# mrjoshuak/go-jpeg2000

Hardware: AMD Instinct MI355X
Metric: Mpixels/s encode+decode (4K sRGB, 5-3 lossless) (higher is better)
Workload: dtype int32

## Files before the change

### go-jpeg2000_amd/csrc/ht.hip

```cpp
#include <cstdlib>

#include "ht_tables.h"
#include "j2k_internal.h"

namespace j2k {

__device__ __constant__ uint16_t c_vlc_tbl0[1024] = J2K_HT_VLC_TBL0_INIT;
__device__ __constant__ uint16_t c_vlc_tbl1[1024] = J2K_HT_VLC_TBL1_INIT;
__device__ uint16_t g_vlc_enc[2 * 4 * 16];

__global__ void ht_build_enc_table() {
    const int t = threadIdx.x;
    if (t >= 128) return;
    const int initial = t >> 6, context = (t >> 4) & 3, rho = t & 15;
    const uint16_t *tbl = initial ? c_vlc_tbl0 : c_vlc_tbl1;
    uint16_t r = 0x0001;
    for (uint32_t cwd = 0; cwd < 128; cwd++) {
        const uint16_t e = tbl[(context << 7) | cwd];
        if (((e >> 4) & 0xF) == rho && (e & 0xF) > 0) { r = (uint16_t)((cwd << 4) | (e & 0xF)); break; }
    }
    g_vlc_enc[t] = r;
}

__device__ uint16_t g_vlc_pair1[16384];
// ... 813 lines not shown
    for (long i = 0; i < num && size > 0; i++) {
        if (unstuff && pos < len && data[pos] > 0x8F) return false;
        uint32_t b;
        if (size > 0 && pos < len) { b = data[pos]; pos++; size--; } else b = 0xFF;
        if (size == 1) b |= 0x0F;
        unstuff = (b == 0xFF);
    }
    return true;
}

#define HT_WALK_MAX_PAIRS 128
#define HT_DEC_MWORDS (33 * HT_FAST_MAX_SAMPLES / 32 + 8)
#define HT_WALK_REC 132
#define HT_PAIR_SERIAL 0xFFFFFFFFu
#define HT_PAIR_ZERO 0xFFFFFFFEu

__device__ __forceinline__ void wave_sync() {
    __builtin_amdgcn_fence(__ATOMIC_RELEASE, "wavefront");
    __builtin_amdgcn_wave_barrier();
    __builtin_amdgcn_fence(__ATOMIC_ACQUIRE, "wavefront");
}

__device__ __forceinline__ uint32_t get_bits32(const uint32_t *buf, uint32_t bitpos) {
    const uint32_t wd = bitpos >> 5, sh = bitpos & 31;
    const uint64_t two = (uint64_t)buf[wd] | ((uint64_t)buf[wd + 1] << 32);
    return (uint32_t)(two >> sh);
}

__device__ __forceinline__ uint32_t get_bits32_cut(const uint32_t *buf, uint32_t bitpos, uint32_t L) {
    if (bitpos >= L) return 0;
    const uint32_t p = bitpos < (HT_DEC_MWORDS - 2) * 32u ? bitpos : (HT_DEC_MWORDS - 2) * 32u + (bitpos & 31);
    uint32_t v = get_bits32(buf, p);
    if (L - bitpos < 32) v &= (1u << (L - bitpos)) - 1;
    return v;
}

#define HT_VBITS_WORDS 192
#define HT_VROW 193

__global__ __launch_bounds__(256) void ht_vlcprep_kernel(const BlockJob *__restrict__ jobs, int njobs,
                                                         const uint8_t *__restrict__ stream, const uint64_t *__restrict__ offs,
                                                         const uint32_t *__restrict__ lens, uint32_t *__restrict__ vbits,
                                                         uint32_t *__restrict__ pairs) {
    __shared__ uint32_t vb4[4][HT_VBITS_WORDS + 8];
    uint32_t *vb = vb4[threadIdx.x >> 6];
    const int jid = blockIdx.x * 4 + (threadIdx.x >> 6);
    if (jid >= njobs) return;
    const int lane = threadIdx.x & 63;
    const int w = jobs[jid].w, h = jobs[jid].h;
    const long len = (long)lens[jid];
    const uint8_t *data = stream + offs[jid];
    uint32_t *rec = pairs + (size_t)jid * HT_WALK_REC;
    const int quadCols = (w + 3) / 4, P = (quadCols + 1) / 2, R = (h + 3) / 4, N = R * P;
    const bool fast = (size_t)R * (size_t)w <= HT_FAST_MAX_SAMPLES && N <= HT_WALK_MAX_PAIRS;
    uint32_t tag = 0;
    long scup = 0;
    if (!fast) tag = HT_PAIR_SERIAL;
    else if (len < 2) tag = HT_PAIR_ZERO;
    else {
        scup = (long)data[len - 1] + ((long)(data[len - 2] & 0x0F) << 8);
        if (scup < 2 || scup > len) tag = HT_PAIR_ZERO;
        else if (!init_mel_ok(data, len, len, scup)) tag = HT_PAIR_ZERO;
    }
    if (tag) {
        if (lane == 0) { rec[0] = tag; rec[HT_WALK_MAX_PAIRS] = 0; }
        return;
    }
    for (int i = lane; i < HT_VBITS_WORDS + 8; i += 64) vb[i] = 0;
    wave_sync();
    const long lcup = len;
    const uint32_t b0 = data[lcup - 2];
    const uint32_t t0 = b0 >> 4;
    uint32_t off = 4 - ((t0 & 7) >> 2);
    if (lane == 0) atomicOr(&vb[0], t0);
    const long size = scup - 2;
    const long maxbytes = (long)(46 * N + 7) / 8 + 8;
    const long nb = size < maxbytes ? size : maxbytes;
    uint32_t carry = b0 | 0x0F;
    for (long k0 = 1; k0 <= nb; k0 += 256) {
        const long k = k0 + 4 * lane;
        const long e = lcup - 2 - k;
        uint32_t dw = 0;
// ... 76 lines not shown
#pragma unroll
        for (int j = 0; j < 8; j++) reinterpret_cast<uint4 *>(S.pair1)[j * 256 + tid] = t[j];
#pragma unroll
        for (int j = 0; j < NV; j++) {
            const int q = j * 256 + tid;
            uint32_t *d = &S.vb[q / 48][4 * (q % 48)];
            d[0] = v[j].x; d[1] = v[j].y; d[2] = v[j].z; d[3] = v[j].w;
        }
    }
    __syncthreads();
#ifdef J2K_WALK_STAMP
    const long long st1 = __builtin_amdgcn_s_memtime();
#endif
    if (tid >= 64) return;
    const int quadCols = (w + 3) / 4, P = (quadCols + 1) / 2, R = (h + 3) / 4;
    const bool walks = have && tag != HT_PAIR_SERIAL && tag != HT_PAIR_ZERO;
    int nsteps = walks ? R * P : 0;
#pragma unroll
    for (int o = 32; o > 0; o >>= 1) nsteps = max(nsteps, __shfl_xor(nsteps, o));
    nsteps = min(__builtin_amdgcn_readfirstlane(nsteps), HT_WALK_MAX_PAIRS);
    if (!walks) return;
    const uint32_t *row = &S.vb[lane][0];
    uint32_t pos = 0;
#define HT_FETCH(w0, w1)                                                          \
    uint32_t w0, w1;                                                               \
    {                                                                              \
        const uint32_t *p_ = row + (pos >> 5);                                     \
        const uint32_t d0_ = p_[0], d1_ = p_[1], d2_ = p_[2];                      \
        w0 = __builtin_amdgcn_alignbit(d1_, d0_, pos & 31);                        \
        w1 = __builtin_amdgcn_alignbit(d2_, d1_, pos & 31);                        \
    }
// ... 64 lines not shown
};

__device__ uint32_t ht_loaded_bits(const HtDecShared &S, uint32_t nff, long segLen, uint32_t j) {
    const long k = 4 * (long)j;
    const long kk = k < segLen ? k : segLen;
    uint32_t f = 0, last_ff = 0;
    for (uint32_t i = 0; i < nff; i++) {
        if ((long)S.ffpos[i] + 2 <= kk) f++;
        if ((long)S.ffpos[i] == segLen - 1) last_ff = 1;
    }
    uint32_t b = (uint32_t)(8 * kk) - f;
    if (k > segLen) b += (last_ff ? 7u : 8u) + 7u * (uint32_t)(k - segLen - 1);
    return b;
}

template <bool STRIDED>
__device__ bool ht_extract_fast(HtDecShared &S, const uint8_t *__restrict__ data, long len, long scup, int w, int h,
                                int32_t *__restrict__ out, int lane, bool bigu, const uint32_t (&mpos2)[2], uint32_t total_bits,
                                const uint32_t (&raw0)[4], int os_) {
    const size_t os64 = STRIDED ? (size_t)os_ : (size_t)64, osw = STRIDED ? (size_t)os_ : (size_t)w;
    const int quadCols = (w + 3) / 4, P = (quadCols + 1) / 2, R = (h + 3) / 4, N = R * P;
    const long lcup = len;
    {
        const long segLen0 = lcup - scup;
        const long cap0 = (long)HT_DEC_MWORDS * 4 - 16;
        const uint32_t zw = bigu ? (uint32_t)HT_DEC_MWORDS
                                 : min((uint32_t)HT_DEC_MWORDS, (uint32_t)(((segLen0 < cap0 ? segLen0 : cap0) * 8) >> 5) + 3u);
        for (uint32_t i = lane; i < zw; i += 64) S.mbuf[i] = 0;
    }
    if (lane == 0) S.nff = 0;
    wave_sync();
    constexpr int PF = 4;
    {
        const long segLen = lcup - scup;
// ... 152 lines not shown
        if (w == 64 && (((uintptr_t)out) & 15) == 0 && (!STRIDED || (os_ & 3) == 0)) {
#pragma unroll
            for (int half = 0; half < 2; half++) {
                const int drow = half * 4 + (lane >> 4), q = lane & 15;
                const int src = drow * 8 + (q >> 1);
                int o[4];
#pragma unroll
                for (int i = 0; i < 4; i++) {
                    const int a = __shfl(vals[i], src), b = __shfl(vals[4 + i], src);
                    o[i] = (q & 1) ? b : a;
                }
                const int rg = 8 * t + drow;
#ifdef J2K_DEC_NO_CODED_STORES
                if (o[0] == 0x7fffffff)
#endif
                if (rg < R) st_decoded(out + (size_t)(4 * rg) * os64 + 4 * q, o[0], o[1], o[2], o[3]);
            }
        } else if (it < N) {
            const int xb = pi * 8;
            int32_t *orow = out + (size_t)(4 * r) * osw + xb;
            if (xb + 8 <= w && (((uintptr_t)orow) & 15) == 0) {
                st_decoded(orow, vals[0], vals[1], vals[2], vals[3]);
                st_decoded(orow + 4, vals[4], vals[5], vals[6], vals[7]);
            } else {
#pragma unroll
                for (int i = 0; i < 8; i++)
                    if (xb + i < w) orow[i] = vals[i];
            }
        }
    }
    return true;
}

template <bool STRIDED>
__global__ __launch_bounds__(256) __attribute__((amdgpu_waves_per_eu(7, 8))) void ht_decode_kernel(const BlockJob *__restrict__ jobs, int njobs,
                                                        const uint8_t *__restrict__ stream, const uint64_t *__restrict__ offs,
                                                        const uint32_t *__restrict__ lens, int32_t *__restrict__ decoded,
                                                        const uint32_t *__restrict__ pairs, int coded_rows_only_) {
    const int coded_rows_only = STRIDED ? 1 : coded_rows_only_;
    __shared__ HtDecShared S4[4];
    HtDecShared &S = S4[threadIdx.x >> 6];
    const int jid = blockIdx.x * 4 + (threadIdx.x >> 6);
    if (jid >= njobs) return;
    const int lane = threadIdx.x & 63;
#ifdef J2K_DEC_STAMP
    const long long d0 = wall_clock64();
#endif
    const BlockJob J = jobs[jid];
    const int w = J.w, h = J.h;
    const int os_ = STRIDED ? J.stride : w;
    int32_t *out = decoded + J.out_off;
    const size_t n = (size_t)w * h;
    const uint32_t *rec = pairs + (size_t)jid * HT_WALK_REC;
    const uint32_t r0 = rec[lane], r1 = rec[64 + lane];
    const uint64_t my_off = offs[jid];
    const uint32_t my_len = lens[jid], my_scup = rec[HT_WALK_MAX_PAIRS];
    const uint32_t tag = __shfl(r0, 0);
    const bool fast = (tag != HT_PAIR_ZERO) && (tag != HT_PAIR_SERIAL);
    auto zero_fill = [&](bool skip_coded) {
        if (coded_rows_only) {
            if (skip_coded) return;
            const uint32_t uw = (uint32_t)w, nrow = (uint32_t)(h + 3) >> 2;
            for (uint32_t i = lane; i < uw * nrow; i += 64) out[(size_t)(i / uw) * 4 * (STRIDED ? (uint32_t)os_ : uw) + i % uw] = 0;
            return;
        }
        if (w == 64 && (J.out_off & 3) == 0) {
            if (skip_coded && lane < 16) return;
            int32_t *q = out + 4 * (size_t)lane;
            for (int i = 0; i < h / 4; i++) st_decoded(q + 256 * (size_t)i, 0, 0, 0, 0);
            const int rem = h & 3;
            if (lane < 16 * rem) st_decoded(q + 256 * (size_t)(h / 4), 0, 0, 0, 0);
        } else if ((w & 3) == 0 && (J.out_off & 3) == 0) {
// ... 9 lines not shown
            const uint32_t uw = (uint32_t)w;
            const uint32_t dy = 64u / uw, dx = 64u % uw;
            uint32_t y = (uint32_t)lane / uw, x = (uint32_t)lane % uw;
            for (uint32_t i = lane; i < (uint32_t)n; i += 64) {
                if (!skip_coded || (y & 3)) out[i] = 0;
                y += dy; x += dx;
                if (x >= uw) { x -= uw; y++; }
            }
        }
    };
    if (!fast) zero_fill(false);
    uint32_t raw0[4] = {0, 0, 0, 0};
#ifdef J2K_DEC_STAMP
    const long long d_a = wall_clock64();
#endif
    if (fast) {
        const uint8_t *fdata = stream + my_off;
        const long segLen = (long)my_len - (long)my_scup;
        const long maxbytes = (long)HT_DEC_MWORDS * 4 - 16;
        const long nb = segLen < maxbytes ? segLen : maxbytes;
        const long d = (long)((uintptr_t)fdata & 3);
        const uint32_t *wsrc = reinterpret_cast<const uint32_t *>(fdata - d);
        const long ndw = (d + nb + 3) >> 2;
        if (ndw > 0) {
#pragma unroll
            for (int c = 0; c < 4; c++) {
                const long j = 64 * c + lane;
                raw0[c] = wsrc[j < ndw ? j : ndw - 1];
            }
        }
        zero_fill(true);
#ifdef J2K_DEC_ONLY_ZERO
        return;
#endif
    }
#ifdef J2K_DEC_STAMP
    const long long d_b = wall_clock64();
#endif
    bool bigu = false;
    uint32_t mpos2[2] = {0, 0}, total_bits = 0;
    {
        const int quadCols = (w + 3) / 4, P = (quadCols + 1) / 2, N = ((h + 3) / 4) * P;
        uint32_t rr[2] = {r0, r1};
#pragma unroll
// ... 10 lines not shown
            if (it < N && (u0 > 31 || u1 > 31)) bigu = true;
            S.pair[it] = (r & 0xFF) | (u0 & 0x3F) << 8 | (u1 & 0x3F) << 14;
            uint32_t nbits = 0;
            if (it < N) {
                const int pi = it % P, xb = pi * 8;
                const uint32_t m1 = (xb + 4 <= w) ? 0xFu : ((xb < w) ? ((1u << (w - xb)) - 1) : 0u);
                const uint32_t m2 = (xb + 8 <= w) ? 0xFu : ((xb + 4 < w) ? ((1u << (w - xb - 4)) - 1) : 0u);
                nbits = __popc(r & 0xF & m1) * ((u0 & 0x3F) + 1) + __popc((r >> 4) & 0xF & m2) * ((u1 & 0x3F) + 1);
            }
            const uint32_t ns = wave_incl_scan(nbits);
            mpos2[t] = total_bits + ns - nbits;
            total_bits += wave_last(ns);
        }
        bigu = __any(bigu);
    }
    wave_sync();
#ifdef J2K_DEC_STAMP
    const long long d_c = wall_clock64();
#endif
#ifdef J2K_DEC_STOP_A
    if (total_bits != 0x7fffffff) return;
#endif
    if (tag == HT_PAIR_ZERO) return;
    if (tag != HT_PAIR_SERIAL) {
        const uint8_t *fdata = stream + my_off;
        const long flen = (long)my_len;
        const long fscup = (long)my_scup;
        if (ht_extract_fast<STRIDED>(S, fdata, flen, fscup, w, h, out, lane, bigu, mpos2, total_bits, raw0, os_)) {
#ifdef J2K_DEC_STAMP
            if ((jid % 700) == 13 && lane == 0) printf("dec job %d: start %lld | job+records %lld | prefetch+zero issue %lld | uvlc+pos %lld | unstuff %lld | extract %lld | end %lld (x10 ns)\n", jid, d0 % 100000, d_a - d0, d_b - d_a, d_c - d_b, g_dbg_unstuff - d_c, wall_clock64() - g_dbg_unstuff, wall_clock64() % 100000);
#endif
            return;
        }
        zero_fill(false);
    }
    __builtin_amdgcn_fence(__ATOMIC_SEQ_CST, "workgroup");
    __builtin_amdgcn_wave_barrier();
    if (lane != 0) return;
    const uint8_t *data = stream + offs[jid];
    const long len = (long)lens[jid];
    if (len < 2) return;
    const long scup = (long)data[len - 1] + ((long)(data[len - 2] & 0x0F) << 8);
    if (scup < 2 || scup > len) return;
// ... 100 lines not shown

hipError_t launch_ht_encode_stream(hipStream_t s, const BlockJob *jobs, int njobs, const int32_t *coef, uint8_t *stream,
                                   uint64_t *offs, uint32_t *lens, uint8_t *numbps, uint64_t *status, uint32_t epoch, int *fault) {
    if (njobs <= 0) return hipSuccess;
    hipError_t e;
    if ((e = ht_tables_ready(s)) != hipSuccess) return e;
    hipLaunchKernelGGL(ht_encode_stream_kernel, dim3(njobs), dim3(64), 0, s, jobs, njobs, coef, stream,
                       reinterpret_cast<unsigned long long *>(offs), lens, numbps, reinterpret_cast<unsigned long long *>(status), epoch, fault);
    return hipGetLastError();
}
int ht_fast_max_samples() { return HT_FAST_MAX_SAMPLES; }

size_t ht_decode_scratch_words(int njobs) { return (size_t)njobs * (HT_WALK_REC + HT_VBITS_WORDS); }

hipError_t launch_ht_decode(hipStream_t s, const BlockJob *jobs, int njobs, const uint8_t *stream, const uint64_t *offs,
                            const uint32_t *lens, int32_t *decoded, uint32_t *scratch, int coded_rows_only, const BlockJob *placed_jobs) {
    if (njobs <= 0) return hipSuccess;
    hipError_t e;
    if ((e = ht_tables_ready(s)) != hipSuccess) return e;
    uint32_t *pairs = scratch, *vbits = scratch + (size_t)njobs * HT_WALK_REC;
    for (int rep_ = 0; rep_ < dev_reps(32); rep_++)
    hipLaunchKernelGGL(ht_vlcprep_kernel, dim3((njobs + 3) / 4), dim3(256), 0, s, jobs, njobs, stream, offs, lens, vbits, pairs);
    if ((e = hipGetLastError()) != hipSuccess) return e;
    for (int rep_ = 0; rep_ < dev_reps(64); rep_++)
    hipLaunchKernelGGL(ht_walk_kernel, dim3((njobs + HT_WALK_BLOCKS - 1) / HT_WALK_BLOCKS), dim3(256), sizeof(HtWalkShared), s, jobs, njobs, vbits, pairs);
    if ((e = hipGetLastError()) != hipSuccess) return e;
    for (int rep_ = 0; rep_ < dev_reps(128); rep_++)
    if (placed_jobs) hipLaunchKernelGGL(ht_decode_kernel<true>, dim3((njobs + 3) / 4), dim3(256), 0, s, placed_jobs, njobs, stream, offs, lens, decoded, pairs, 1);
    else
    hipLaunchKernelGGL(ht_decode_kernel<false>, dim3((njobs + 3) / 4), dim3(256), 0, s, jobs, njobs, stream, offs, lens, decoded, pairs, coded_rows_only);
    return hipGetLastError();
}

}
```

### go-jpeg2000_amd/csrc/j2k_ctx.cpp

```cpp
#include "j2k_host.h"

using namespace j2k;

int fail(j2k_ctx *ctx, int status, const char *msg) {
    if (ctx) ctx->last_error = msg ? msg : "";
    return status;
}
int fail_hip(j2k_ctx *ctx, hipError_t e, const char *where) {
    char buf[256];
    snprintf(buf, sizeof(buf), "%s: %s", where, hipGetErrorString(e));
    if (ctx) ctx->last_error = buf;
    return J2K_ERR_HIP;
}

extern "C" const char *j2k_ctx_last_error(j2k_ctx *ctx) { return ctx ? ctx->last_error.c_str() : ""; }

std::atomic<int> g_mq_ctxs{0};
bool mq_throughput_mode() { return g_mq_ctxs.load(std::memory_order_relaxed) >= 2; }
struct CtxOption { const char *name; bool (*set)(j2k_ctx *, long); };
static const std::vector<CtxOption> &ctx_options() {
#define OPT(name, cond, stmt) CtxOption{name, [](j2k_ctx *c, long v) -> bool { (void)c; if (!(cond)) return false; stmt; return true; }}
    static const std::vector<CtxOption> T = {
        OPT("plane_wg3", v == 0 || v == 1, c->plane_wg3 = v != 0),
        OPT("pix_fuse", v >= 0 && v <= 2, c->pix_fuse = (int)v),
        OPT("plane_wg", v == 0 || v == 4 || v == 8, c->plane_wg = (int)v),
        OPT("l0_fuse", v == 0 || v == 8 || v == 10 || v == 16, c->l0_fuse = (int)v),
        OPT("l0_wg", v == 0 || v == 4 || v == 8, c->l0_wg = (int)v),
        OPT("plane_wg97", v == 0 || v == 8, c->plane_wg97 = (int)v),
        OPT("l0_wg97_inv", v == 0 || v == 6 || v == 8 || v == 10 || v == 12, c->l0_wg97_inv = (int)v),
        OPT("l0_wg97", v == 0 || (v >= 6 && v <= 16 && v % 2 == 0), c->l0_wg97 = (int)v),
        OPT("l0_xcd", v == 0 || v == 1, c->l0_xcd = v != 0),
        OPT("l0_deal", v == 0 || v == 1, c->l0_deal = v != 0),
        OPT("ht_alias", v == 0 || v == 1, c->ht_alias = v != 0),
        OPT("l0_inv_wpe", v >= 5 && v <= 7, c->l0_inv_wpe = (int)v),
        OPT("l0_wg_inv", v == 0 || v == 1, c->l0_wg_inv = v != 0),
        OPT("l0_wg_invw", v == 0 || v == 4 || v == 8, c->l0_wg_invw = (int)v),
        OPT("l0_xcd_group", v >= 0 && v <= 4096, c->l0_xcd_group = (int)v),
        OPT("l0_store", v == 0 || v == 1 || v == 2 || v == 4, c->l0_store = (int)v),
        OPT("fuse_compact", v == 0 || v == 1, c->fuse_compact = v != 0),
        OPT("deep", v == 0 || v == 1, c->use_deep = v != 0),
        OPT("deep_min_planes", v >= 0 && v <= 1000000, c->deep_min_planes = (int)v),
        OPT("deep_mid", v == 0 || v == 1, c->deep_mid = v != 0),
        OPT("deep_mid_inv", v >= 0 && v <= 2, c->deep_mid_inv = (int)v),
        OPT("mega", v >= 0 && v <= 2, c->mega = (int)v),
        OPT("t1_split", v == 0 || v == 1, c->t1_split = v != 0),
        OPT("t1_sym_mb", v >= 0, c->t1_sym_mb = v),
        OPT("t1_dec_general", v == 0 || v == 1, c->t1_dec_general = v != 0),
        OPT("t1_dec_split", v >= -1, c->t1_dec_split = (int)v),
// ... 126 lines not shown
    for (size_t i = 0; i + 1 < ctx->ev_used; i += 2) {
        if (ctx->ev_tag[i / 2] != 0) continue;
        float ms = 0;
        HIPCHK(ctx, hipEventElapsedTime(&ms, ctx->ev[i], ctx->ev[i + 1]));
        tot += ms; n++;
    }
    *launches = n;
    *total_ms = tot;
    ctx->ev_used = 0;
    return J2K_OK;
}
extern "C" int j2k_ctx_profile_read_tag(j2k_ctx *ctx, int tag, int64_t *launches, double *total_ms) {
    if (!ctx || !launches || !total_ms) return J2K_ERR_INVALID_ARG;
    HIPCHK(ctx, hipSetDevice(ctx->device));
    HIPCHK(ctx, hipStreamSynchronize(ctx->stream));
    double tot = 0;
    int64_t n = 0;
    for (size_t i = 0; i + 1 < ctx->ev_used; i += 2) {
        if (ctx->ev_tag[i / 2] != tag) continue;
        float ms = 0;
        HIPCHK(ctx, hipEventElapsedTime(&ms, ctx->ev[i], ctx->ev[i + 1]));
        tot += ms; n++;
    }
    *launches = n;
    *total_ms = tot;
    return J2K_OK;
}
static hipEvent_t profile_event(j2k_ctx *ctx) {
    if (!ctx->profile || ctx->capturing || ctx->ev_used >= 8192) return nullptr;
    if (ctx->ev_used >= ctx->ev.size()) {
// ... 35 lines not shown
```

### go-jpeg2000_amd/csrc/j2k_host.h

```cpp
#pragma once
#include <algorithm>
#include <atomic>
#include <cstdio>
#include <cstdlib>
#include <cstring>
#include <map>
#include <tuple>

#include "j2k_plan.h"

namespace j2k {
#ifdef J2K_DEV
int g_dev_skip = 0, g_dev_dup = 0;
#endif
hipError_t launch_add_const(hipStream_t s, int32_t *d, size_t n, int delta);
hipError_t launch_rct(hipStream_t s, int32_t *a, int32_t *b, int32_t *c, size_t n, int inverse);
hipError_t launch_ict(hipStream_t s, double *a, double *b, double *c, size_t n, int inverse);
hipError_t launch_dwt97_fwd(hipStream_t s, const LevelLaunch &L, const void *src, int src_is_f64, int32_t *out_i32,
                            double *out_f64, double *nxt, int dc_shift, int quant, double step, int mct);
hipError_t launch_dwt97_inv(hipStream_t s, const LevelLaunch &L, const void *coef, int coef_is_f64, const double *prev,
                            void *dst, int dc_shift, int final_level, int dst_mode, int mct);
hipError_t launch_ht_encode(hipStream_t s, const BlockJob *jobs, int njobs, const int32_t *coef, uint8_t *slots,
                            uint32_t *lens, uint8_t *numbps, int *fault, uint32_t *maglens = nullptr, const HtUJob *utab = nullptr, int nunique = 0,
                            const int *alias_ids = nullptr);
hipError_t launch_ht_decode(hipStream_t s, const BlockJob *jobs, int njobs, const uint8_t *stream, const uint64_t *offs,
                            const uint32_t *lens, int32_t *decoded, uint32_t *scratch, int coded_rows_only = 0, const BlockJob *placed_jobs = nullptr);
size_t ht_decode_scratch_words(int njobs);
hipError_t launch_ht_encode_stream(hipStream_t s, const BlockJob *jobs, int njobs, const int32_t *coef, uint8_t *stream,
                                   uint64_t *offs, uint32_t *lens, uint8_t *numbps, uint64_t *status, uint32_t epoch, int *fault);
int ht_fast_max_samples();
hipError_t launch_t1_encode(hipStream_t s, const BlockJob *jobs, int njobs, const int32_t *coef, uint8_t *slots,
                            uint32_t *lens, uint8_t *numbps, uint8_t *work, size_t work_per_job, int *fault, int max_dim,
                            uint8_t *sym, size_t sym_stride, uint32_t *nsyms, int lanes, uint8_t *bigsym = nullptr, const uint64_t *bigsym_off = nullptr,
                            uint32_t *bignsyms = nullptr);
size_t t1_sym_stride(int planes);
hipError_t launch_t1_decode(hipStream_t s, const BlockJob *jobs, int njobs, const uint8_t *stream, const uint64_t *offs,
                            const uint32_t *lens, const uint8_t *numbps, int32_t *decoded, uint8_t *work,
                            size_t work_per_job, int max_dim, int general_only, uint8_t *split_ws, int sig_lanes, int throughput = 0);
size_t t1_dec_split_bytes(size_t njobs);
hipError_t launch_mq_encode(hipStream_t s, const uint8_t *ctxs, const uint8_t *decs, size_t n, uint8_t *out, size_t cap, uint32_t *out_len, int *fault);
hipError_t launch_mq_decode(hipStream_t s, const uint8_t *data, size_t len, const uint8_t *ctxs, size_t n, uint8_t *decs, int *fault);
// ... 71 lines not shown
```

### go-jpeg2000_amd/csrc/j2k_internal.h

```cpp
#pragma once
#include <hip/hip_runtime.h>
#include <stdint.h>
#include <stdlib.h>
#include <algorithm>
#include "../../include/j2kgfx.h"
#include "image_color.h"

namespace j2k {

struct DwtPlane {
    int64_t src_off[3];
    int64_t out_off[3];
    int64_t nxt_off[3];
    int32_t src_stride;
    int32_t w, h;
    int32_t n_next;
    int32_t out_stride;
    int32_t pad_;
};

struct DwtJob {
    int32_t plane;
    int32_t col0;
    int32_t prow0;
// ... 1 lines not shown
};
#define J2K_LINK_UP 0x10000
#define J2K_LINK_DOWN 0x20000

struct BlockJob {
    int64_t src_off;
    int64_t out_off;
    int32_t stride;
    int32_t w, h;
    int32_t band;
};

struct HtUJob {
    BlockJob J;
    int32_t jid;
    int32_t alias_off;
    int32_t nalias;
    int32_t pad_;
};

struct TailPlane {
    int64_t scr_off;
    int64_t coef_off;
    int32_t w, h;
    int32_t nlev;
    int32_t pad_;
};

struct YccSrc {
    const uint8_t *y, *cb, *cr;
// ... 111 lines not shown
```

### go-jpeg2000_amd/csrc/j2k_plan.h

```cpp
#pragma once
#include <string>
#include <vector>

#include "../../include/j2kgfx.h"
#include "j2k_internal.h"

struct j2k_ctx {
    int device = -1;
    hipStream_t stream = nullptr;
    std::string last_error;
    int fuse_compact = 0;
    int fwd_link = 1;
    int inv_link = 1;
    int pix_fuse = 1;
    bool plane_wg3 = false;
    int plane_wg = 4;
    int l0_fuse = 0;
    int l0_wg = 8;
    int l0_wg_invw = 4;
    bool l0_deal = true;
    int l0_wg97 = 8;
    int plane_wg97 = 8;
    int l0_wg97_inv = 8;
    int l0_xcd_group = 16;
    bool l0_xcd = true;
    bool ht_alias = true;
    int l0_inv_wpe = 5;
    bool l0_wg_inv = true;
    int l0_store = 1;
    int band_prows_pix = 3;
    int band_prows_97 = 8;
    int band_prows_inv = 0;
    int fwd_pf = 0;
    int band_prows = 5;
    int use_tail = 1;
    int mega = 0;
    int deep_mid_inv = 1;
    int deep_min_planes = 12;
    int deep_mid = 1;
    int use_deep = 1;
    int xcd_map = 0;
// ... 5 lines not shown
    int t1_dec_lanes = 2;
    int t1_dec_split = -1;
    bool capturing = false;
    bool fault_armed_before_capture = false;
    bool counted_mq = false;
    bool t2_parallel = true;
    int t1_lanes = 0;
    std::vector<j2k_plan *> cache;
    void *stage[5] = {nullptr, nullptr, nullptr, nullptr, nullptr};
    bool fault_armed = false;
    size_t stage_bytes[5] = {0, 0, 0, 0, 0};
    int profile = 0;
    std::vector<hipEvent_t> ev;
    std::vector<int> ev_tag;
    size_t ev_used = 0;
};

namespace j2k {

enum Wavelet { W53 = 0, W97 = 1 };
enum QuantMode {
    Q_NONE = 0,
    Q_ENCODER = 1,
    Q_TCD = 2
};

struct PlanSpec {
    int W = 0, H = 0, C = 1;
    int tile_w = 0, tile_h = 0;
    int levels = 1;
// ... 82 lines not shown
    size_t host_io_bytes = 0, host_pix_bytes = 0;
    int *d_tile_job0 = nullptr;
    uint64_t max_tile_bytes = 0;
    std::vector<uint64_t> slot_off;
    std::vector<uint64_t> dec_off;
    j2k::BlockJob *d_bjobs = nullptr;
    j2k::BlockJob *d_djobs = nullptr;
    j2k::BlockJob *d_djobs_placed = nullptr;
    int64_t bytes_cap = 0, decoded_elems = 0, block_samples = 0;
    int64_t dwt_bytes = 0, dwt_level0_bytes = 0;
    void *d_frame = nullptr, *d_coeff = nullptr, *d_slots = nullptr, *d_stream = nullptr;
    void *d_lens = nullptr, *d_numbps = nullptr, *d_offs = nullptr;
    j2k::DwtJob *d_fwd_pix_jobs = nullptr;
    int fwd_pix_njobs = 0;
    j2k::HtUJob *d_ht_ujobs = nullptr; int *d_ht_alias_next = nullptr;
    j2k::BlockJob *d_bjobs_alias = nullptr;
    int ht_nunique = 0;
    j2k::DwtJob *d_fwd97_wg_jobs = nullptr;
    int fwd97_wg_njobs = 0, fwd97_wg_waves = 0;
    j2k::DwtJob *d_inv97_wg_jobs = nullptr;
    int inv97_wg_njobs = 0, inv97_wg_waves = 0;
    j2k::DwtJob *d_fwd_wg2_jobs = nullptr, *d_fwd_wg_rest_jobs = nullptr;
    int fwd_wg2_njobs = 0, fwd_wg2_waves = 0, fwd_wg_rest_njobs = 0;
    j2k::DwtJob *d_fwd_wg_jobs = nullptr;
    int fwd_wg_njobs = 0, fwd_wg_waves = 0;
    j2k::DwtJob *d_inv_wg_jobs = nullptr;
    int inv_wg_njobs = 0, inv_wg_waves = 0;
    uint32_t *d_maglens = nullptr;
    uint32_t *d_mels = nullptr;
    const void *last_stream = nullptr, *last_lens = nullptr;
// ... 10 lines not shown
```

### go-jpeg2000_amd/csrc/j2k_planbuild.cpp

```cpp
#include "j2k_host.h"

using namespace j2k;

bool PlanSpec::operator==(const PlanSpec &o) const {
    return W == o.W && H == o.H && C == o.C && tile_w == o.tile_w && tile_h == o.tile_h && levels == o.levels &&
           frame_h == o.frame_h && wavelet == o.wavelet && precision == o.precision && dc_shift == o.dc_shift && dc_shift_inv == o.dc_shift_inv && mct == o.mct && quant == o.quant && quality == o.quality &&
           num_res_jobs == o.num_res_jobs && cb_w == o.cb_w && cb_h == o.cb_h && coder == o.coder &&
           tile_first == o.tile_first && tile_count == o.tile_count && frame_is_f64 == o.frame_is_f64 && closed_loop == o.closed_loop;
}

static inline int pick_cpl(int maxw) { return maxw >= 384 ? 8 : (maxw >= 192 ? 4 : 2); }

extern "C" size_t j2k_block_bound(int coder, int w, int h) {
    size_t n = (size_t)std::max(w, 0) * (size_t)std::max(h, 0);
    if (coder == J2K_CODER_HT) {
        size_t maxSize = std::max<size_t>(n * 2, 64);
        return maxSize / 2 + maxSize / 4 + maxSize / 2 + 2;
    }
    return std::max<size_t>(n * 2 + 1024, 16384);
}


static void make_jobs(std::vector<DwtJob> &jobs, int plane, int w, int h, int cpl, int band, int halo) {
    const int halfH = (h + 1) / 2;
// ... 570 lines not shown
                auto it = first.find(key);
                if (it == first.end()) { first[key] = (int)ujobs.size(); ujobs.push_back((int)i); lists.push_back({(int)i}); }
                else { lists[it->second].push_back((int)i); aj[i].out_off = bj[ujobs[it->second]].out_off; }
            }
            if (ujobs.size() < bj.size()) {
                std::vector<HtUJob> utab;
                std::vector<int> ids;
                for (size_t u = 0; u < ujobs.size(); u++) {
                    utab.push_back(HtUJob{bj[ujobs[u]], ujobs[u], (int)ids.size(), (int)lists[u].size(), 0});
                    ids.insert(ids.end(), lists[u].begin(), lists[u].end());
                }
                P->ht_nunique = (int)ujobs.size();
                r = upload(ctx, &P->d_ht_ujobs, utab);
                if (r == J2K_OK) r = upload(ctx, &P->d_ht_alias_next, ids);
                if (r == J2K_OK) r = upload(ctx, &P->d_bjobs_alias, aj);
            }
        }
        for (size_t i = 0; i < bj.size(); i++) bj[i].out_off = (int64_t)P->dec_off[i];
        if (r == J2K_OK) r = upload(ctx, &P->d_djobs, bj);
        if (r == J2K_OK && P->spec.closed_loop && P->spec.coder == J2K_CODER_HT) {
            for (size_t i = 0; i < bj.size(); i++) bj[i].out_off = bj[i].src_off;
            r = upload(ctx, &P->d_djobs_placed, bj);
        }
        if (r != J2K_OK) { j2k_plan_destroy(P); return r; }
    }
    *out = P;
    return J2K_OK;
}

extern "C" void j2k_plan_destroy(j2k_plan *P) {
    if (!P) return;
    if (P->ctx) { (void)hipSetDevice(P->ctx->device); (void)hipStreamSynchronize(P->ctx->stream); }
    for (int cls = 0; cls < 2; cls++) {
        for (auto &T : P->fwd[cls]) { if (T.d_planes) (void)hipFree(T.d_planes); if (T.d_jobs) (void)hipFree(T.d_jobs); if (T.d_pjobs) (void)hipFree(T.d_pjobs); }
        if (cls == 0 && P->d_bigsym_off) { (void)hipFree(P->d_bigsym_off); P->d_bigsym_off = nullptr; }
        for (auto &T : P->inv[cls]) { if (T.d_planes) (void)hipFree(T.d_planes); if (T.d_jobs) (void)hipFree(T.d_jobs); if (T.d_pjobs) (void)hipFree(T.d_pjobs); }
    }
    void *ptrs[] = {P->d_deep_jobs_inv, P->d_mega_fwd_jobs, P->d_mega_inv_jobs, P->d_fwd_top_jobs, P->d_inv_top_jobs, P->d_inv_wg_jobs, P->d_deep_planes, P->d_deep_jobs, P->d_tile_job0, P->d_scrA, P->d_scrB, P->d_tail, P->d_bjobs, P->d_djobs, P->d_djobs_placed, P->d_frame, P->d_coeff, P->d_slots, P->d_stream, P->d_lens, P->d_numbps, P->d_offs, P->d_status, P->d_fwd_pix_jobs, P->d_fwd_wg2_jobs, P->d_fwd_wg_rest_jobs, P->d_fwd_wg_jobs, P->d_fwd97_wg_jobs, P->d_inv97_wg_jobs, P->d_ht_ujobs, P->d_ht_alias_next, P->d_bjobs_alias, P->d_maglens, P->d_mels, P->d_toffs,
                    P->d_t2_packets, P->d_tile_packet0, P->d_t2_cbs, P->d_t2_poffs, P->d_t2_ptile, P->d_t2_ws, P->d_t2_chains, P->d_t2_body_base, P->d_t2_par, P->d_frame_status,
                    P->d_cl_decoded, P->d_cl_coeff, P->d_cl_coeff_dec, P->d_cl_numbps, P->d_cl_offs, P->d_cl_lens, P->d_host_io, P->d_host_pix};
    for (void *p : ptrs) if (p) (void)hipFree(p);
    delete P;
}

static int spec_from_params(j2k_ctx *ctx, const j2k_params *p, PlanSpec &S) {
    if (!p) return fail(ctx, J2K_ERR_INVALID_ARG, "params == NULL");
    if (p->precision < 1 || p->precision > 31) return fail(ctx, J2K_ERR_INVALID_ARG, "precision out of range");
    S.W = p->width; S.H = p->height; S.C = p->ncomp;
    S.frame_h = p->frame_rows > 0 ? p->frame_rows : p->height;
    if (S.frame_h > 0 && p->height % S.frame_h) return fail(ctx, J2K_ERR_INVALID_ARG, "height is not a whole number of frames (frame_rows)");
    S.tile_w = p->tile_w; S.tile_h = p->tile_h;
    S.levels = p->num_resolutions - 1;
    if (S.levels <= 0) S.levels = 5;
// ... 54 lines not shown
```

### go-jpeg2000_amd/csrc/j2k_stages.cpp

```cpp
#include "j2k_host.h"

using namespace j2k;

static LevelLaunch mk(const LevelTab &T, int pf = 0) {
    LevelLaunch L{T.d_jobs, T.njobs, T.d_planes, T.cpl, T.vec, T.ncomp, pf};
    L.pjobs = T.d_pjobs; L.pnjobs = T.p_pix_only ? 0 : T.pnjobs; L.pwaves = T.pwaves; L.pmulti = T.pmulti;
    return L;
}

static void pix_launch(LevelLaunch &L, const LevelTab &T, const PixIO &pix, int cls, const PlanSpec &S) {
    L.pix_stride = pix.stride;
    L.pix_src = cls ? (pix.triple == 4 ? 4 : 0) : pix.single;
    L.comp_elems = (long long)S.W * S.H;
    if (cls == 1 && pix.triple == 4) L.pnjobs = T.pnjobs;
}

int plan_forward_impl(j2k_plan *P, const void *d_frame, void *d_coeff, PixIO pix) {
    const int pix_stride = pix.stride;
    j2k_ctx *ctx = P->ctx;
    const PlanSpec &S = P->spec;
    if (((uintptr_t)d_frame & 15) || ((uintptr_t)d_coeff & 15)) return fail(ctx, J2K_ERR_INVALID_ARG, "device pointers must be 16-byte aligned");
    HIPCHK(ctx, hipSetDevice(ctx->device));
    const double step = 1.0 / (double)S.quality;
    const int nlevel_launches = (P->deep_l0 >= 0) ? P->deep_l0 : ((P->tail_l0 >= 0) ? P->tail_l0 : S.levels);
// ... 648 lines not shown
    P->dec_coded_rows_only = on != 0;
    return J2K_OK;
}

extern "C" int j2k_plan_decode_blocks(j2k_plan *P, const uint8_t *d_stream, const uint64_t *d_offs, const uint32_t *d_lens,
                                      const uint8_t *d_numbps, int32_t *d_decoded) {
    if (!P || !d_stream || !d_offs || !d_lens || !d_numbps || !d_decoded) return J2K_ERR_INVALID_ARG;
    j2k_ctx *ctx = P->ctx;
    HIPCHK(ctx, hipSetDevice(ctx->device));
    const int n = (int)P->blocks.size();
    if (!n) return J2K_OK;
    if (P->spec.coder == J2K_CODER_HT) {
        int r = stage_reserve(ctx, 2, ht_decode_scratch_words(n) * 4 + 256);
        if (r != J2K_OK) return r;
        HIPCHK(ctx, launch_ht_decode(ctx->stream, P->d_djobs, n, d_stream, d_offs, d_lens, d_decoded, (uint32_t *)ctx->stage[2],
                                     P->dec_coded_rows_only ? 1 : 0));
    } else {
        size_t wpj = 0;
        int max_dim = 0;
        for (const j2k_block &b : P->blocks) { wpj = std::max(wpj, t1_flag_bytes(b.w, b.h)); max_dim = std::max(max_dim, std::max(b.w, b.h)); }
        wpj = (wpj + 255) & ~size_t(255);
        const int split_min = ctx->t1_dec_split >= 0 ? ctx->t1_dec_split : (mq_throughput_mode() ? 512 : 12000);
        bool split = split_min > 0 && n >= split_min && !ctx->t1_dec_general && !((uintptr_t)d_stream & 15);
        const size_t gen_bytes = (wpj * (size_t)n + 255) & ~size_t(255);
        int r = stage_reserve(ctx, 2, gen_bytes + 256 + (split ? j2k::t1_dec_split_bytes((size_t)n) : 0));
        if (r != J2K_OK && split) { (void)hipGetLastError(); split = false; r = stage_reserve(ctx, 2, gen_bytes + 256); }
        if (r != J2K_OK) return r;
        HIPCHK(ctx, launch_t1_decode(ctx->stream, P->d_djobs, n, d_stream, d_offs, d_lens, d_numbps, d_decoded,
                                     (uint8_t *)ctx->stage[2], wpj, max_dim, ctx->t1_dec_general,
                                     split ? (uint8_t *)ctx->stage[2] + gen_bytes : nullptr, ctx->t1_dec_lanes, mq_throughput_mode() ? 1 : 0));
    }
// ... 4 lines not shown
```

Measured before the change: 76980.

## Deduplicate HT decode of byte-identical code blocks via leader fan-out stores

Before decoding, the prep kernel compares each HT code block's bytes with the leader of its encode-side alias group and tags it ALIAS when they match. Aliased blocks skip their own VLC walk and decode. The leader's wave writes its decoded samples to every aliased output location. This removes redundant entropy decoding when the frame holds many identical code blocks, at the cost of a full byte comparison per aliased block and serialized extra stores in the leader's wave. A host-side alias counter is also added as a debug query.

Result: no change. 77490, median of 6 (+0.7%).

```diff
diff --git a/go-jpeg2000_amd/csrc/ht.hip b/go-jpeg2000_amd/csrc/ht.hip
--- a/go-jpeg2000_amd/csrc/ht.hip
+++ b/go-jpeg2000_amd/csrc/ht.hip
@@ -1,4 +1,5 @@
 #include <cstdlib>
+#include <vector>
 
 #include "ht_tables.h"
 #include "j2k_internal.h"
@@ -851,6 +852,7 @@
 #define HT_WALK_REC 132
 #define HT_PAIR_SERIAL 0xFFFFFFFFu
 #define HT_PAIR_ZERO 0xFFFFFFFEu
+#define HT_PAIR_ALIAS 0xFFFFFFFDu
 
 __device__ __forceinline__ void wave_sync() {
     __builtin_amdgcn_fence(__ATOMIC_RELEASE, "wavefront");
@@ -878,7 +880,7 @@
 __global__ __launch_bounds__(256) void ht_vlcprep_kernel(const BlockJob *__restrict__ jobs, int njobs,
                                                          const uint8_t *__restrict__ stream, const uint64_t *__restrict__ offs,
                                                          const uint32_t *__restrict__ lens, uint32_t *__restrict__ vbits,
-                                                         uint32_t *__restrict__ pairs) {
+                                                         uint32_t *__restrict__ pairs, const HtDecAlias *__restrict__ dalias) {
     __shared__ uint32_t vb4[4][HT_VBITS_WORDS + 8];
     uint32_t *vb = vb4[threadIdx.x >> 6];
     const int jid = blockIdx.x * 4 + (threadIdx.x >> 6);
@@ -903,6 +905,31 @@
         if (lane == 0) { rec[0] = tag; rec[HT_WALK_MAX_PAIRS] = 0; }
         return;
     }
+    if (dalias) {
+        const int lead = dalias[jid].leader;
+        if (lead != jid && (long)lens[lead] == len) {
+            const uint8_t *ld = stream + offs[lead];
+            bool diff = false;
+            if (len >= 16) {
+                for (long i0 = 0; i0 < len; i0 += 4096) {
+                    uint4 a[4], b[4];
+#pragma unroll
+                    for (int c = 0; c < 4; c++) {
+                        long i = i0 + 1024 * c + 16 * lane;
+                        if (i > len - 16) i = len - 16;
+                        __builtin_memcpy(&a[c], data + i, 16);
+                        __builtin_memcpy(&b[c], ld + i, 16);
+                    }
+#pragma unroll
+                    for (int c = 0; c < 4; c++) diff |= ((a[c].x ^ b[c].x) | (a[c].y ^ b[c].y) | (a[c].z ^ b[c].z) | (a[c].w ^ b[c].w)) != 0;
+                }
+            } else if (lane < len) diff = data[lane] != ld[lane];
+            if (!__any(diff)) {
+                if (lane == 0) { rec[0] = HT_PAIR_ALIAS; rec[HT_WALK_MAX_PAIRS] = (uint32_t)scup; }
+                return;
+            }
+        }
+    }
     for (int i = lane; i < HT_VBITS_WORDS + 8; i += 64) vb[i] = 0;
     wave_sync();
     const long lcup = len;
@@ -1009,7 +1036,7 @@
 #endif
     if (tid >= 64) return;
     const int quadCols = (w + 3) / 4, P = (quadCols + 1) / 2, R = (h + 3) / 4;
-    const bool walks = have && tag != HT_PAIR_SERIAL && tag != HT_PAIR_ZERO;
+    const bool walks = have && tag != HT_PAIR_SERIAL && tag != HT_PAIR_ZERO && tag != HT_PAIR_ALIAS;
     int nsteps = walks ? R * P : 0;
 #pragma unroll
     for (int o = 32; o > 0; o >>= 1) nsteps = max(nsteps, __shfl_xor(nsteps, o));
@@ -1104,10 +1131,38 @@
     return b;
 }
 
+struct HtDecTargets {
+    int32_t *decoded;
+    const BlockJob *jobs;
+    const uint32_t *pairs;
+    const int *ids;
+    int n;
+    long long off0;
+};
+__device__ __forceinline__ long long ht_target_off(const HtDecTargets &T, int k) {
+    if (k < 1 || k >= T.n) return -1;
+    const int m = T.ids[k];
+    return T.pairs[(size_t)m * HT_WALK_REC] == HT_PAIR_ALIAS ? (long long)T.jobs[m].out_off : -1;
+}
+
 template <bool STRIDED>
 __device__ bool ht_extract_fast(HtDecShared &S, const uint8_t *__restrict__ data, long len, long scup, int w, int h,
                                 int32_t *__restrict__ out, int lane, bool bigu, const uint32_t (&mpos2)[2], uint32_t total_bits,
-                                const uint32_t (&raw0)[4], int os_) {
+                                const uint32_t (&raw0)[4], int os_, const HtDecTargets &T) {
+    auto each_block = [&](auto &&store) {
+        store(out);
+        if constexpr (!STRIDED) {
+            for (int k0 = 0; k0 < T.n; k0 += 64) {
+                const long long mo = k0 == 0 ? T.off0 : ht_target_off(T, k0 + lane);
+                unsigned long long m = __ballot(mo >= 0);
+                while (m) {
+                    const int k = __ffsll((long long)m) - 1;
+                    m &= m - 1;
+                    store(T.decoded + __shfl(mo, k));
+                }
+            }
+        }
+    };
     const size_t os64 = STRIDED ? (size_t)os_ : (size_t)64, osw = STRIDED ? (size_t)os_ : (size_t)w;
     const int quadCols = (w + 3) / 4, P = (quadCols + 1) / 2, R = (h + 3) / 4, N = R * P;
     const long lcup = len;
@@ -1290,19 +1345,24 @@
 #ifdef J2K_DEC_NO_CODED_STORES
                 if (o[0] == 0x7fffffff)
 #endif
-                if (rg < R) st_decoded(out + (size_t)(4 * rg) * os64 + 4 * q, o[0], o[1], o[2], o[3]);
-            }
-        } else if (it < N) {
+                each_block([&](int32_t *blk) {
+                    if (rg < R) st_decoded(blk + (size_t)(4 * rg) * os64 + 4 * q, o[0], o[1], o[2], o[3]);
+                });
+            }
+        } else {
             const int xb = pi * 8;
-            int32_t *orow = out + (size_t)(4 * r) * osw + xb;
-            if (xb + 8 <= w && (((uintptr_t)orow) & 15) == 0) {
-                st_decoded(orow, vals[0], vals[1], vals[2], vals[3]);
-                st_decoded(orow + 4, vals[4], vals[5], vals[6], vals[7]);
-            } else {
-#pragma unroll
-                for (int i = 0; i < 8; i++)
-                    if (xb + i < w) orow[i] = vals[i];
-            }
+            each_block([&](int32_t *blk) {
+                if (it >= N) return;
+                int32_t *orow = blk + (size_t)(4 * r) * osw + xb;
+                if (xb + 8 <= w && (((uintptr_t)orow) & 15) == 0) {
+                    st_decoded(orow, vals[0], vals[1], vals[2], vals[3]);
+                    st_decoded(orow + 4, vals[4], vals[5], vals[6], vals[7]);
+                } else {
+#pragma unroll
+                    for (int i = 0; i < 8; i++)
+                        if (xb + i < w) orow[i] = vals[i];
+                }
+            });
         }
     }
     return true;
@@ -1312,7 +1372,8 @@
 __global__ __launch_bounds__(256) __attribute__((amdgpu_waves_per_eu(7, 8))) void ht_decode_kernel(const BlockJob *__restrict__ jobs, int njobs,
                                                         const uint8_t *__restrict__ stream, const uint64_t *__restrict__ offs,
                                                         const uint32_t *__restrict__ lens, int32_t *__restrict__ decoded,
-                                                        const uint32_t *__restrict__ pairs, int coded_rows_only_) {
+                                                        const uint32_t *__restrict__ pairs, int coded_rows_only_,
+                                                        const HtDecAlias *__restrict__ dalias, const int *__restrict__ alias_ids) {
     const int coded_rows_only = STRIDED ? 1 : coded_rows_only_;
     __shared__ HtDecShared S4[4];
     HtDecShared &S = S4[threadIdx.x >> 6];
@@ -1328,10 +1389,18 @@
     int32_t *out = decoded + J.out_off;
     const size_t n = (size_t)w * h;
     const uint32_t *rec = pairs + (size_t)jid * HT_WALK_REC;
-    const uint32_t r0 = rec[lane], r1 = rec[64 + lane];
+    uint32_t r0 = rec[lane], r1 = rec[64 + lane];
     const uint64_t my_off = offs[jid];
     const uint32_t my_len = lens[jid], my_scup = rec[HT_WALK_MAX_PAIRS];
-    const uint32_t tag = __shfl(r0, 0);
+    HtDecAlias A{jid, 0, 0, 0};
+    if (!STRIDED && dalias) A = dalias[jid];
+    uint32_t tag = __shfl(r0, 0);
+    const bool alias = !STRIDED && tag == HT_PAIR_ALIAS;
+    if (alias) {
+        const uint32_t *lrec = pairs + (size_t)A.leader * HT_WALK_REC;
+        r0 = lrec[lane]; r1 = lrec[64 + lane];
+        tag = 0;
+    }
     const bool fast = (tag != HT_PAIR_ZERO) && (tag != HT_PAIR_SERIAL);
     auto zero_fill = [&](bool skip_coded) {
         if (coded_rows_only) {
@@ -1371,7 +1440,8 @@
 #ifdef J2K_DEC_STAMP
     const long long d_a = wall_clock64();
 #endif
-    if (fast) {
+    HtDecTargets T{decoded, jobs, pairs, alias_ids + A.alias_off, 0, -1};
+    auto fetch_raw0 = [&]() {
         const uint8_t *fdata = stream + my_off;
         const long segLen = (long)my_len - (long)my_scup;
         const long maxbytes = (long)HT_DEC_MWORDS * 4 - 16;
@@ -1385,6 +1455,12 @@
                 const long j = 64 * c + lane;
                 raw0[c] = wsrc[j < ndw ? j : ndw - 1];
             }
+        }
+    };
+    if (fast) {
+        if (!alias) {
+            fetch_raw0();
+            if (!STRIDED && A.nalias > 1 && A.leader == jid) { T.n = A.nalias; T.off0 = ht_target_off(T, lane); }
         }
         zero_fill(true);
 #ifdef J2K_DEC_ONLY_ZERO
@@ -1425,6 +1501,11 @@
         }
         bigu = __any(bigu);
     }
+    if (!STRIDED) {
+        if (alias && !bigu) return;
+        if (bigu) T.n = 0;
+        if (alias) fetch_raw0();
+    }
     wave_sync();
 #ifdef J2K_DEC_STAMP
     const long long d_c = wall_clock64();
@@ -1437,7 +1518,7 @@
         const uint8_t *fdata = stream + my_off;
         const long flen = (long)my_len;
         const long fscup = (long)my_scup;
-        if (ht_extract_fast<STRIDED>(S, fdata, flen, fscup, w, h, out, lane, bigu, mpos2, total_bits, raw0, os_)) {
+        if (ht_extract_fast<STRIDED>(S, fdata, flen, fscup, w, h, out, lane, bigu, mpos2, total_bits, raw0, os_, T)) {
 #ifdef J2K_DEC_STAMP
             if ((jid % 700) == 13 && lane == 0) printf("dec job %d: start %lld | job+records %lld | prefetch+zero issue %lld | uvlc+pos %lld | unstuff %lld | extract %lld | end %lld (x10 ns)\n", jid, d0 % 100000, d_a - d0, d_b - d_a, d_c - d_b, g_dbg_unstuff - d_c, wall_clock64() - g_dbg_unstuff, wall_clock64() % 100000);
 #endif
@@ -1568,22 +1649,34 @@
 size_t ht_decode_scratch_words(int njobs) { return (size_t)njobs * (HT_WALK_REC + HT_VBITS_WORDS); }
 
 hipError_t launch_ht_decode(hipStream_t s, const BlockJob *jobs, int njobs, const uint8_t *stream, const uint64_t *offs,
-                            const uint32_t *lens, int32_t *decoded, uint32_t *scratch, int coded_rows_only, const BlockJob *placed_jobs) {
+                            const uint32_t *lens, int32_t *decoded, uint32_t *scratch, int coded_rows_only, const BlockJob *placed_jobs,
+                            const HtDecAlias *dalias, const int *alias_ids) {
     if (njobs <= 0) return hipSuccess;
     hipError_t e;
     if ((e = ht_tables_ready(s)) != hipSuccess) return e;
     uint32_t *pairs = scratch, *vbits = scratch + (size_t)njobs * HT_WALK_REC;
     for (int rep_ = 0; rep_ < dev_reps(32); rep_++)
-    hipLaunchKernelGGL(ht_vlcprep_kernel, dim3((njobs + 3) / 4), dim3(256), 0, s, jobs, njobs, stream, offs, lens, vbits, pairs);
+    hipLaunchKernelGGL(ht_vlcprep_kernel, dim3((njobs + 3) / 4), dim3(256), 0, s, jobs, njobs, stream, offs, lens, vbits, pairs, placed_jobs ? nullptr : dalias);
     if ((e = hipGetLastError()) != hipSuccess) return e;
     for (int rep_ = 0; rep_ < dev_reps(64); rep_++)
     hipLaunchKernelGGL(ht_walk_kernel, dim3((njobs + HT_WALK_BLOCKS - 1) / HT_WALK_BLOCKS), dim3(256), sizeof(HtWalkShared), s, jobs, njobs, vbits, pairs);
     if ((e = hipGetLastError()) != hipSuccess) return e;
     for (int rep_ = 0; rep_ < dev_reps(128); rep_++)
-    if (placed_jobs) hipLaunchKernelGGL(ht_decode_kernel<true>, dim3((njobs + 3) / 4), dim3(256), 0, s, placed_jobs, njobs, stream, offs, lens, decoded, pairs, 1);
+    if (placed_jobs) hipLaunchKernelGGL(ht_decode_kernel<true>, dim3((njobs + 3) / 4), dim3(256), 0, s, placed_jobs, njobs, stream, offs, lens, decoded, pairs, 1, nullptr, nullptr);
     else
-    hipLaunchKernelGGL(ht_decode_kernel<false>, dim3((njobs + 3) / 4), dim3(256), 0, s, jobs, njobs, stream, offs, lens, decoded, pairs, coded_rows_only);
+    hipLaunchKernelGGL(ht_decode_kernel<false>, dim3((njobs + 3) / 4), dim3(256), 0, s, jobs, njobs, stream, offs, lens, decoded, pairs, coded_rows_only, dalias, alias_ids);
     return hipGetLastError();
 }
 
-}
+hipError_t ht_decode_count_aliases(hipStream_t s, const uint32_t *scratch, int njobs, long *count) {
+    *count = 0;
+    if (njobs <= 0) return hipSuccess;
+    std::vector<uint32_t> tags((size_t)njobs);
+    hipError_t e = hipStreamSynchronize(s);
+    if (e != hipSuccess) return e;
+    if ((e = hipMemcpy2D(tags.data(), 4, scratch, (size_t)HT_WALK_REC * 4, 4, (size_t)njobs, hipMemcpyDeviceToHost)) != hipSuccess) return e;
+    for (uint32_t t : tags) *count += t == HT_PAIR_ALIAS;
+    return hipSuccess;
+}
+
+}
diff --git a/go-jpeg2000_amd/csrc/j2k_ctx.cpp b/go-jpeg2000_amd/csrc/j2k_ctx.cpp
--- a/go-jpeg2000_amd/csrc/j2k_ctx.cpp
+++ b/go-jpeg2000_amd/csrc/j2k_ctx.cpp
@@ -32,6 +32,7 @@
         OPT("l0_xcd", v == 0 || v == 1, c->l0_xcd = v != 0),
         OPT("l0_deal", v == 0 || v == 1, c->l0_deal = v != 0),
         OPT("ht_alias", v == 0 || v == 1, c->ht_alias = v != 0),
+        OPT("ht_dec_alias", v == 0 || v == 1, c->ht_dec_alias = v != 0),
         OPT("l0_inv_wpe", v >= 5 && v <= 7, c->l0_inv_wpe = (int)v),
         OPT("l0_wg_inv", v == 0 || v == 1, c->l0_wg_inv = v != 0),
         OPT("l0_wg_invw", v == 0 || v == 4 || v == 8, c->l0_wg_invw = (int)v),
@@ -188,6 +189,13 @@
     if (!ctx || !launches || !total_ms) return J2K_ERR_INVALID_ARG;
     HIPCHK(ctx, hipSetDevice(ctx->device));
     HIPCHK(ctx, hipStreamSynchronize(ctx->stream));
+    if (tag == 16) {
+        long c = 0;
+        HIPCHK(ctx, ht_decode_count_aliases(ctx->stream, (const uint32_t *)ctx->stage[2], ctx->stage[2] ? ctx->ht_dec_last_blocks : 0, &c));
+        *launches = c;
+        *total_ms = 0;
+        return J2K_OK;
+    }
     double tot = 0;
     int64_t n = 0;
     for (size_t i = 0; i + 1 < ctx->ev_used; i += 2) {
diff --git a/go-jpeg2000_amd/csrc/j2k_host.h b/go-jpeg2000_amd/csrc/j2k_host.h
--- a/go-jpeg2000_amd/csrc/j2k_host.h
+++ b/go-jpeg2000_amd/csrc/j2k_host.h
@@ -24,7 +24,9 @@
                             uint32_t *lens, uint8_t *numbps, int *fault, uint32_t *maglens = nullptr, const HtUJob *utab = nullptr, int nunique = 0,
                             const int *alias_ids = nullptr);
 hipError_t launch_ht_decode(hipStream_t s, const BlockJob *jobs, int njobs, const uint8_t *stream, const uint64_t *offs,
-                            const uint32_t *lens, int32_t *decoded, uint32_t *scratch, int coded_rows_only = 0, const BlockJob *placed_jobs = nullptr);
+                            const uint32_t *lens, int32_t *decoded, uint32_t *scratch, int coded_rows_only = 0, const BlockJob *placed_jobs = nullptr,
+                            const HtDecAlias *dalias = nullptr, const int *alias_ids = nullptr);
+hipError_t ht_decode_count_aliases(hipStream_t s, const uint32_t *scratch, int njobs, long *count);
 size_t ht_decode_scratch_words(int njobs);
 hipError_t launch_ht_encode_stream(hipStream_t s, const BlockJob *jobs, int njobs, const int32_t *coef, uint8_t *stream,
                                    uint64_t *offs, uint32_t *lens, uint8_t *numbps, uint64_t *status, uint32_t epoch, int *fault);
diff --git a/go-jpeg2000_amd/csrc/j2k_internal.h b/go-jpeg2000_amd/csrc/j2k_internal.h
--- a/go-jpeg2000_amd/csrc/j2k_internal.h
+++ b/go-jpeg2000_amd/csrc/j2k_internal.h
@@ -39,6 +39,13 @@
 struct HtUJob {
     BlockJob J;
     int32_t jid;
+    int32_t alias_off;
+    int32_t nalias;
+    int32_t pad_;
+};
+
+struct HtDecAlias {
+    int32_t leader;
     int32_t alias_off;
     int32_t nalias;
     int32_t pad_;
diff --git a/go-jpeg2000_amd/csrc/j2k_plan.h b/go-jpeg2000_amd/csrc/j2k_plan.h
--- a/go-jpeg2000_amd/csrc/j2k_plan.h
+++ b/go-jpeg2000_amd/csrc/j2k_plan.h
@@ -25,6 +25,7 @@
     int l0_xcd_group = 16;
     bool l0_xcd = true;
     bool ht_alias = true;
+    bool ht_dec_alias = true;
     int l0_inv_wpe = 5;
     bool l0_wg_inv = true;
     int l0_store = 1;
@@ -60,6 +61,7 @@
     std::vector<hipEvent_t> ev;
     std::vector<int> ev_tag;
     size_t ev_used = 0;
+    int ht_dec_last_blocks = 0;
 };
 
 namespace j2k {
@@ -172,6 +174,7 @@
     j2k::DwtJob *d_fwd_pix_jobs = nullptr;
     int fwd_pix_njobs = 0;
     j2k::HtUJob *d_ht_ujobs = nullptr; int *d_ht_alias_next = nullptr;
+    j2k::HtDecAlias *d_ht_dalias = nullptr;
     j2k::BlockJob *d_bjobs_alias = nullptr;
     int ht_nunique = 0;
     j2k::DwtJob *d_fwd97_wg_jobs = nullptr;
diff --git a/go-jpeg2000_amd/csrc/j2k_planbuild.cpp b/go-jpeg2000_amd/csrc/j2k_planbuild.cpp
--- a/go-jpeg2000_amd/csrc/j2k_planbuild.cpp
+++ b/go-jpeg2000_amd/csrc/j2k_planbuild.cpp
@@ -608,6 +608,16 @@
                 r = upload(ctx, &P->d_ht_ujobs, utab);
                 if (r == J2K_OK) r = upload(ctx, &P->d_ht_alias_next, ids);
                 if (r == J2K_OK) r = upload(ctx, &P->d_bjobs_alias, aj);
+                if (r == J2K_OK && ctx->ht_dec_alias) {
+                    std::vector<HtDecAlias> da(bj.size());
+                    bool aligned = true;
+                    for (size_t u = 0; u < ujobs.size(); u++)
+                        for (size_t k = 0; k < lists[u].size(); k++) {
+                            da[lists[u][k]] = HtDecAlias{ujobs[u], k ? 0 : utab[u].alias_off, k ? 0 : utab[u].nalias, 0};
+                            aligned = aligned && (P->dec_off[lists[u][k]] & 3) == 0;
+                        }
+                    if (aligned) r = upload(ctx, &P->d_ht_dalias, da);
+                }
             }
         }
         for (size_t i = 0; i < bj.size(); i++) bj[i].out_off = (int64_t)P->dec_off[i];
@@ -630,7 +640,7 @@
         if (cls == 0 && P->d_bigsym_off) { (void)hipFree(P->d_bigsym_off); P->d_bigsym_off = nullptr; }
         for (auto &T : P->inv[cls]) { if (T.d_planes) (void)hipFree(T.d_planes); if (T.d_jobs) (void)hipFree(T.d_jobs); if (T.d_pjobs) (void)hipFree(T.d_pjobs); }
     }
-    void *ptrs[] = {P->d_deep_jobs_inv, P->d_mega_fwd_jobs, P->d_mega_inv_jobs, P->d_fwd_top_jobs, P->d_inv_top_jobs, P->d_inv_wg_jobs, P->d_deep_planes, P->d_deep_jobs, P->d_tile_job0, P->d_scrA, P->d_scrB, P->d_tail, P->d_bjobs, P->d_djobs, P->d_djobs_placed, P->d_frame, P->d_coeff, P->d_slots, P->d_stream, P->d_lens, P->d_numbps, P->d_offs, P->d_status, P->d_fwd_pix_jobs, P->d_fwd_wg2_jobs, P->d_fwd_wg_rest_jobs, P->d_fwd_wg_jobs, P->d_fwd97_wg_jobs, P->d_inv97_wg_jobs, P->d_ht_ujobs, P->d_ht_alias_next, P->d_bjobs_alias, P->d_maglens, P->d_mels, P->d_toffs,
+    void *ptrs[] = {P->d_deep_jobs_inv, P->d_mega_fwd_jobs, P->d_mega_inv_jobs, P->d_fwd_top_jobs, P->d_inv_top_jobs, P->d_inv_wg_jobs, P->d_deep_planes, P->d_deep_jobs, P->d_tile_job0, P->d_scrA, P->d_scrB, P->d_tail, P->d_bjobs, P->d_djobs, P->d_djobs_placed, P->d_frame, P->d_coeff, P->d_slots, P->d_stream, P->d_lens, P->d_numbps, P->d_offs, P->d_status, P->d_fwd_pix_jobs, P->d_fwd_wg2_jobs, P->d_fwd_wg_rest_jobs, P->d_fwd_wg_jobs, P->d_fwd97_wg_jobs, P->d_inv97_wg_jobs, P->d_ht_ujobs, P->d_ht_alias_next, P->d_ht_dalias, P->d_bjobs_alias, P->d_maglens, P->d_mels, P->d_toffs,
                     P->d_t2_packets, P->d_tile_packet0, P->d_t2_cbs, P->d_t2_poffs, P->d_t2_ptile, P->d_t2_ws, P->d_t2_chains, P->d_t2_body_base, P->d_t2_par, P->d_frame_status,
                     P->d_cl_decoded, P->d_cl_coeff, P->d_cl_coeff_dec, P->d_cl_numbps, P->d_cl_offs, P->d_cl_lens, P->d_host_io, P->d_host_pix};
     for (void *p : ptrs) if (p) (void)hipFree(p);
diff --git a/go-jpeg2000_amd/csrc/j2k_stages.cpp b/go-jpeg2000_amd/csrc/j2k_stages.cpp
--- a/go-jpeg2000_amd/csrc/j2k_stages.cpp
+++ b/go-jpeg2000_amd/csrc/j2k_stages.cpp
@@ -686,7 +686,8 @@
         int r = stage_reserve(ctx, 2, ht_decode_scratch_words(n) * 4 + 256);
         if (r != J2K_OK) return r;
         HIPCHK(ctx, launch_ht_decode(ctx->stream, P->d_djobs, n, d_stream, d_offs, d_lens, d_decoded, (uint32_t *)ctx->stage[2],
-                                     P->dec_coded_rows_only ? 1 : 0));
+                                     P->dec_coded_rows_only ? 1 : 0, nullptr, P->d_ht_dalias, P->d_ht_alias_next));
+        ctx->ht_dec_last_blocks = n;
     } else {
         size_t wpj = 0;
         int max_dim = 0;
```
